# MCG-NJU/MeMOTR

Hardware: AMD Instinct MI355X
Metric: train_frames_per_sec (higher is better)
Workload: dtype f32

## Files before the change

### memotr_amd/csrc/clip_ops.hip

```cpp
#include <hip/hip_runtime.h>
#include <stdint.h>
#include <stdio.h>

#include <atomic>

#include "../../include/clip_ops_hip.h"
#include "assign_core.h"

namespace {

thread_local char g_err[256] = {0};

int fail(int code, const char *msg) {
    snprintf(g_err, sizeof(g_err), "%s", msg);
    return code;
}

int check_launch(const char *what) {
    const hipError_t e = hipGetLastError();
    if (e != hipSuccess) {
        snprintf(g_err, sizeof(g_err), "%s: %s", what, hipGetErrorString(e));
        return (int)e;
    }
    g_err[0] = 0;
// ... 330 lines not shown
        a.y += __shfl_xor(a.y, o, 64);
        a.z += __shfl_xor(a.z, o, 64);
        a.w += __shfl_xor(a.w, o, 64);
    }
    if ((threadIdx.x & 63) == 0) s_w[threadIdx.x >> 6] = a;
    __syncthreads();
    if (threadIdx.x == 0) *reinterpret_cast<f32x4_t *>(out + c) = (s_w[0] + s_w[1]) + (s_w[2] + s_w[3]);
}

__device__ __forceinline__ float colsum_ld(const float *x, long i) { return x[i]; }
__device__ __forceinline__ float colsum_ld(const uint16_t *x, long i) {
    return __uint_as_float(((unsigned)x[i]) << 16);
}

template <typename TX>
__global__ __launch_bounds__(256) void colsum_partial_kernel(const TX *__restrict__ x, long rows, int cols,
                                                            int chunk_rows, float *__restrict__ partial) {
    __shared__ float s_part[8][33];
    const int tx = threadIdx.x & 31, ty = threadIdx.x >> 5;
    const int c = blockIdx.x * 32 + tx;
    const long r0 = (long)blockIdx.y * chunk_rows;
    const long r1 = r0 + chunk_rows < rows ? r0 + chunk_rows : rows;
    float a0 = 0.f, a1 = 0.f, a2 = 0.f, a3 = 0.f;
    if (c < cols) {
        long r = r0 + ty;
        for (; r + 24 < r1; r += 32) {
            a0 += colsum_ld(x, r * cols + c);
            a1 += colsum_ld(x, (r + 8) * cols + c);
            a2 += colsum_ld(x, (r + 16) * cols + c);
            a3 += colsum_ld(x, (r + 24) * cols + c);
        }
        for (; r < r1; r += 8) a0 += colsum_ld(x, r * cols + c);
    }
    s_part[ty][tx] = (a0 + a1) + (a2 + a3);
    __syncthreads();
    if (ty == 0 && c < cols) {
        float t = s_part[0][tx];
#pragma unroll
        for (int i = 1; i < 8; ++i) t += s_part[i][tx];
        partial[(long)blockIdx.y * cols + c] = t;
    }
}

__device__ __forceinline__ void colsum_st(float *x, long i, float v) { x[i] = v; }

template <typename TX>
__global__ __launch_bounds__(256) void relu_bwd_colsum_partial_kernel(const TX *__restrict__ g, const TX *__restrict__ y,
                                                                     long rows, int cols, int chunk_rows,
                                                                     TX *__restrict__ g2, float *__restrict__ partial) {
    __shared__ float s_part[8][33];
    const int tx = threadIdx.x & 31, ty = threadIdx.x >> 5;
    const int c = blockIdx.x * 32 + tx;
    const long r0 = (long)blockIdx.y * chunk_rows;
    const long r1 = r0 + chunk_rows < rows ? r0 + chunk_rows : rows;
    float a0 = 0.f, a1 = 0.f, a2 = 0.f, a3 = 0.f;
    if (c < cols) {
        long r = r0 + ty;
        for (; r + 24 < r1; r += 32) {
            const long i0 = r * cols + c, i1 = (r + 8) * cols + c, i2 = (r + 16) * cols + c, i3 = (r + 24) * cols + c;
            const float v0 = colsum_ld(y, i0) <= 0.f ? 0.f : colsum_ld(g, i0);
            const float v1 = colsum_ld(y, i1) <= 0.f ? 0.f : colsum_ld(g, i1);
            const float v2 = colsum_ld(y, i2) <= 0.f ? 0.f : colsum_ld(g, i2);
            const float v3 = colsum_ld(y, i3) <= 0.f ? 0.f : colsum_ld(g, i3);
            colsum_st(g2, i0, v0); colsum_st(g2, i1, v1); colsum_st(g2, i2, v2); colsum_st(g2, i3, v3);
            a0 += v0; a1 += v1; a2 += v2; a3 += v3;
        }
        for (; r < r1; r += 8) {
            const long i0 = r * cols + c;
            const float v0 = colsum_ld(y, i0) <= 0.f ? 0.f : colsum_ld(g, i0);
            colsum_st(g2, i0, v0);
            a0 += v0;
        }
    }
    s_part[ty][tx] = (a0 + a1) + (a2 + a3);
    __syncthreads();
    if (ty == 0 && c < cols) {
        float t = s_part[0][tx];
#pragma unroll
        for (int i = 1; i < 8; ++i) t += s_part[i][tx];
        partial[(long)blockIdx.y * cols + c] = t;
    }
}

constexpr int kLanes = 16;
constexpr int kRows = 256 / kLanes;
constexpr int kHd = 32;
constexpr int kPitch = 36;

__device__ __forceinline__ void load_row32(const float *p, float *r) {
#pragma unroll
    for (int i = 0; i < 8; ++i) {
        const f32x4_t v = *reinterpret_cast<const f32x4_t *>(p + 4 * i);
        r[4 * i] = v.x; r[4 * i + 1] = v.y; r[4 * i + 2] = v.z; r[4 * i + 3] = v.w;
    }
}

__device__ __forceinline__ float dot32(const float *a, const float *lds_row) {
    float s0 = 0.f, s1 = 0.f;
#pragma unroll
    for (int i = 0; i < 8; ++i) {
        const f32x4_t v = *reinterpret_cast<const f32x4_t *>(lds_row + 4 * i);
        s0 = fmaf(a[4 * i], v.x, s0);
        s1 = fmaf(a[4 * i + 1], v.y, s1);
        s0 = fmaf(a[4 * i + 2], v.z, s0);
        s1 = fmaf(a[4 * i + 3], v.w, s1);
    }
    return s0 + s1;
}

__device__ __forceinline__ void axpy32(float *acc, float w, const float *lds_row) {
#pragma unroll
    for (int i = 0; i < 8; ++i) {
        const f32x4_t v = *reinterpret_cast<const f32x4_t *>(lds_row + 4 * i);
        acc[4 * i] = fmaf(w, v.x, acc[4 * i]);
        acc[4 * i + 1] = fmaf(w, v.y, acc[4 * i + 1]);
        acc[4 * i + 2] = fmaf(w, v.z, acc[4 * i + 2]);
        acc[4 * i + 3] = fmaf(w, v.w, acc[4 * i + 3]);
    }
}

__device__ __forceinline__ float sum8l(float x) {
#pragma unroll
    for (int o = 1; o < kLanes; o <<= 1) x += __shfl_xor(x, o, 64);
    return x;
}
__device__ __forceinline__ float max8l(float x) {
#pragma unroll
    for (int o = 1; o < kLanes; o <<= 1) x = fmaxf(x, __shfl_xor(x, o, 64));
    return x;
}

__device__ __forceinline__ void stage_rows(float *dst, const float *src, long rs, int L) {
    for (int i = threadIdx.x; i < L * 8; i += blockDim.x) {
        const int r = i >> 3, c = (i & 7) * 4;
        *reinterpret_cast<f32x4_t *>(dst + r * kPitch + c) = *reinterpret_cast<const f32x4_t *>(src + r * rs + c);
    }
}

__global__ __launch_bounds__(256) void mha_fwd_kernel(const float *__restrict__ q, const float *__restrict__ k,
                                                     const float *__restrict__ v, long q_bs, long q_rs, long k_bs,
                                                     long k_rs, long v_bs, long v_rs,
                                                     const uint8_t *__restrict__ key_mask, int H, int L, float scale,
                                                     float *__restrict__ out, float *__restrict__ lse) {
    extern __shared__ __attribute__((aligned(16))) float s_mem[];
    float *Ks = s_mem, *Vs = s_mem + (size_t)L * kPitch;
    const int h = blockIdx.y, b = blockIdx.z;
    stage_rows(Ks, k + b * k_bs + h * kHd, k_rs, L);
    stage_rows(Vs, v + b * v_bs + h * kHd, v_rs, L);
    __syncthreads();
    const int row = blockIdx.x * kRows + threadIdx.x / kLanes, sub = threadIdx.x % kLanes;
    const bool row_ok = row < L;
    const int rowc = row_ok ? row : L - 1;
    float qr[kHd];
    load_row32(q + b * q_bs + rowc * q_rs + h * kHd, qr);
#pragma unroll
    for (int i = 0; i < kHd; ++i) qr[i] *= scale;
    const uint8_t *mk = key_mask ? key_mask + (long)b * L : nullptr;
    float m = -INFINITY, l = 0.f, acc[kHd];
#pragma unroll
    for (int i = 0; i < kHd; ++i) acc[i] = 0.f;
    for (int j = sub; j < L; j += kLanes) {
        if (mk && mk[j]) continue;
        const float s = dot32(qr, Ks + j * kPitch);
        const float m_new = fmaxf(m, s);
        const float corr = expf(m - m_new), p = expf(s - m_new);
        l = l * corr + p;
#pragma unroll
        for (int i = 0; i < kHd; ++i) acc[i] *= corr;
        axpy32(acc, p, Vs + j * kPitch);
        m = m_new;
    }
    const float M = max8l(m);
    const float w = (m == -INFINITY) ? 0.f : expf(m - M);
    const float Lsum = sum8l(l * w);
    const float inv = 1.f / Lsum;
    float *o = out + ((long)b * L + rowc) * (H * kHd) + h * kHd;
#pragma unroll
    for (int i = 0; i < kHd; ++i) {
        const float t = sum8l(acc[i] * w) * inv;
        if (row_ok && (i >> 2) == sub) o[i] = t;
    }
    if (row_ok && sub == 0) lse[((long)b * H + h) * L + row] = M + logf(Lsum);
}

__global__ __launch_bounds__(256) void mha_bwd_q_kernel(const float *__restrict__ q, const float *__restrict__ k,
                                                       const float *__restrict__ v, long q_bs, long q_rs, long k_bs,
                                                       long k_rs, long v_bs, long v_rs,
                                                       const uint8_t *__restrict__ key_mask,
                                                       const float *__restrict__ out, const float *__restrict__ lse,
                                                       const float *__restrict__ go, int H, int L, float scale,
                                                       float *__restrict__ gq, long gq_bs, long gq_rs) {
    extern __shared__ __attribute__((aligned(16))) float s_mem[];
    float *Ks = s_mem, *Vs = s_mem + (size_t)L * kPitch;
    const int h = blockIdx.y, b = blockIdx.z;
    stage_rows(Ks, k + b * k_bs + h * kHd, k_rs, L);
    stage_rows(Vs, v + b * v_bs + h * kHd, v_rs, L);
    __syncthreads();
    const int row = blockIdx.x * kRows + threadIdx.x / kLanes, sub = threadIdx.x % kLanes;
    const bool row_ok = row < L;
    const int rowc = row_ok ? row : L - 1;
    float qr[kHd], gr[kHd], acc[kHd];
    load_row32(q + b * q_bs + rowc * q_rs + h * kHd, qr);
    const long orow = ((long)b * L + rowc) * (H * kHd) + h * kHd;
    load_row32(go + orow, gr);
    float D = 0.f;
    {
        float orr[kHd];
        load_row32(out + orow, orr);
#pragma unroll
        for (int i = 0; i < kHd; ++i) D = fmaf(gr[i], orr[i], D);
    }
#pragma unroll
    for (int i = 0; i < kHd; ++i) { qr[i] *= scale; acc[i] = 0.f; }
    const float ls = lse[((long)b * H + h) * L + rowc];
    const uint8_t *mk = key_mask ? key_mask + (long)b * L : nullptr;
    for (int j = sub; j < L; j += kLanes) {
        if (mk && mk[j]) continue;
        const float p = expf(dot32(qr, Ks + j * kPitch) - ls);
        const float ds = p * (dot32(gr, Vs + j * kPitch) - D);
        axpy32(acc, ds, Ks + j * kPitch);
    }
    float *g = gq + b * gq_bs + rowc * gq_rs + h * kHd;
#pragma unroll
    for (int i = 0; i < kHd; ++i) {
        const float t = sum8l(acc[i]) * scale;
        if (row_ok && (i >> 2) == sub) g[i] = t;
    }
}

__global__ __launch_bounds__(256) void mha_bwd_kv_kernel(const float *__restrict__ q, const float *__restrict__ k,
                                                        const float *__restrict__ v, long q_bs, long q_rs, long k_bs,
                                                        long k_rs, long v_bs, long v_rs,
                                                        const uint8_t *__restrict__ key_mask,
                                                        const float *__restrict__ out, const float *__restrict__ lse,
                                                        const float *__restrict__ go, int H, int L, float scale,
                                                        float *__restrict__ gk, long gk_bs, long gk_rs,
                                                        float *__restrict__ gv, long gv_bs, long gv_rs) {
    extern __shared__ __attribute__((aligned(16))) float s_mem[];
    float *Qs = s_mem, *Gs = s_mem + (size_t)L * kPitch;
    float *s_lse = Gs + (size_t)L * kPitch, *s_D = s_lse + L;
    const int h = blockIdx.y, b = blockIdx.z;
    stage_rows(Qs, q + b * q_bs + h * kHd, q_rs, L);
    stage_rows(Gs, go + (long)b * L * (H * kHd) + h * kHd, (long)H * kHd, L);
    for (int i = threadIdx.x; i < L; i += blockDim.x) s_lse[i] = lse[((long)b * H + h) * L + i];
    __syncthreads();
    for (int i = threadIdx.x; i < L; i += blockDim.x) {
        const float *o = out + ((long)b * L + i) * (H * kHd) + h * kHd;
        float d = 0.f;
#pragma unroll
        for (int c = 0; c < kHd; ++c) d = fmaf(Gs[i * kPitch + c], o[c], d);
        s_D[i] = d;
    }
    __syncthreads();
    const int row = blockIdx.x * kRows + threadIdx.x / kLanes, sub = threadIdx.x % kLanes;
    const bool row_ok = row < L;
    const int rowc = row_ok ? row : L - 1;
    const bool dead = key_mask && key_mask[(long)b * L + rowc];
    float kr[kHd], vr[kHd], ak[kHd], av[kHd];
    load_row32(k + b * k_bs + rowc * k_rs + h * kHd, kr);
    load_row32(v + b * v_bs + rowc * v_rs + h * kHd, vr);
#pragma unroll
    for (int i = 0; i < kHd; ++i) { kr[i] *= scale; ak[i] = 0.f; av[i] = 0.f; }
    if (!dead) {
        for (int i = sub; i < L; i += kLanes) {
            const float p = expf(dot32(kr, Qs + i * kPitch) - s_lse[i]);
            const float ds = p * (dot32(vr, Gs + i * kPitch) - s_D[i]);
            axpy32(av, p, Gs + i * kPitch);
            axpy32(ak, ds, Qs + i * kPitch);
        }
    }
    float *pk = gk + b * gk_bs + rowc * gk_rs + h * kHd, *pv = gv + b * gv_bs + rowc * gv_rs + h * kHd;
#pragma unroll
    for (int i = 0; i < kHd; ++i) {
        const float tk = sum8l(ak[i]) * scale, tv = sum8l(av[i]);
        if (row_ok && (i >> 2) == sub) {
            pk[i] = tk;
            pv[i] = tv;
        }
    }
}

int allow_lds(const void *kernel, size_t lds, std::atomic<unsigned long long> &done) {
    if (lds <= 64 * 1024) return 0;
    int dev = 0;
    (void)hipGetDevice(&dev);
    const unsigned long long bit = 1ull << (dev & 63);
    if (done.load(std::memory_order_acquire) & bit) return 0;
    const hipError_t e = hipFuncSetAttribute(kernel, hipFuncAttributeMaxDynamicSharedMemorySize, 160 * 1024 - 2048);
    if (e != hipSuccess) {
        snprintf(g_err, sizeof(g_err), "hipFuncSetAttribute: %s", hipGetErrorString(e));
        return (int)e;
    }
    done.fetch_or(bit, std::memory_order_release);
    return 0;
}

std::atomic<unsigned long long> g_lds_fwd{0}, g_lds_bq{0}, g_lds_bkv{0};

int mha_check(const void *q, const void *k, const void *v, int B, int H, int L) {
    if (B < 0 || H <= 0 || L < 0) return fail(1, "clipops_mha: bad dimension");
    if (L > CLIPOPS_MHA_MAX_L) return fail(2, "clipops_mha: L exceeds CLIPOPS_MHA_MAX_L");
    if ((long)B * L > 0 && (!q || !k || !v)) return fail(1, "clipops_mha: null pointer");
    return 0;
}

__device__ __forceinline__ float wave_sum64(float x) {
#pragma unroll
    for (int o = 32; o > 0; o >>= 1) x += __shfl_xor(x, o, 64);
    return x;
}

__global__ __launch_bounds__(256) void add_layer_norm_fwd_kernel(const float *__restrict__ x,
                                                                const float *__restrict__ res,
                                                                const float *__restrict__ gamma,
                                                                const float *__restrict__ beta, long rows, float eps,
                                                                float *__restrict__ sum, float *__restrict__ y,
                                                                float *__restrict__ stats) {
    const int lane = threadIdx.x & 63;
    const long row = (long)blockIdx.x * 4 + (threadIdx.x >> 6);
    if (row >= rows) return;
    const long off = row * CLIPOPS_LN_COLS + lane * 4;
    const f32x4_t a = *reinterpret_cast<const f32x4_t *>(x + off);
    const f32x4_t b = *reinterpret_cast<const f32x4_t *>(res + off);
    const f32x4_t s = a + b;
    *reinterpret_cast<f32x4_t *>(sum + off) = s;
    const float mean = wave_sum64((s.x + s.y) + (s.z + s.w)) * (1.f / CLIPOPS_LN_COLS);
    const f32x4_t d = s - mean;
    const float var = wave_sum64((d.x * d.x + d.y * d.y) + (d.z * d.z + d.w * d.w)) * (1.f / CLIPOPS_LN_COLS);
    const float rstd = rsqrtf(var + eps);
    const f32x4_t g = *reinterpret_cast<const f32x4_t *>(gamma + lane * 4);
    const f32x4_t be = *reinterpret_cast<const f32x4_t *>(beta + lane * 4);
    *reinterpret_cast<f32x4_t *>(y + off) = (d * rstd) * g + be;
    if (lane == 0) {
        stats[2 * row] = mean;
        stats[2 * row + 1] = rstd;
    }
}

__global__ __launch_bounds__(256) void add_layer_norm_bwd_kernel(const float *__restrict__ gy,
                                                                const float *__restrict__ sum,
                                                                const float *__restrict__ stats,
                                                                const float *__restrict__ gamma, long rows,
                                                                int chunk_rows, float *__restrict__ gsum,
                                                                float *__restrict__ partial) {
    __shared__ f32x4_t s_acc[4][2][64];
    const int lane = threadIdx.x & 63, wave = threadIdx.x >> 6;
    const f32x4_t gm = *reinterpret_cast<const f32x4_t *>(gamma + lane * 4);
    f32x4_t acc_g = {0.f, 0.f, 0.f, 0.f}, acc_b = {0.f, 0.f, 0.f, 0.f};
    const long r0 = (long)blockIdx.x * chunk_rows;
    const long r1 = r0 + chunk_rows < rows ? r0 + chunk_rows : rows;
    for (long row = r0 + wave; row < r1; row += 4) {
        const long off = row * CLIPOPS_LN_COLS + lane * 4;
        const f32x4_t g = *reinterpret_cast<const f32x4_t *>(gy + off);
        const f32x4_t s = *reinterpret_cast<const f32x4_t *>(sum + off);
        const float mean = stats[2 * row], rstd = stats[2 * row + 1];
        const f32x4_t xh = (s - mean) * rstd;
        const f32x4_t gh = g * gm;
        const float c1 = wave_sum64((gh.x + gh.y) + (gh.z + gh.w)) * (1.f / CLIPOPS_LN_COLS);
        const float c2 = wave_sum64((gh.x * xh.x + gh.y * xh.y) + (gh.z * xh.z + gh.w * xh.w)) * (1.f / CLIPOPS_LN_COLS);
        *reinterpret_cast<f32x4_t *>(gsum + off) = (gh - c1 - xh * c2) * rstd;
        acc_g += g * xh;
        acc_b += g;
    }
    s_acc[wave][0][lane] = acc_g;
    s_acc[wave][1][lane] = acc_b;
    __syncthreads();
    if (wave < 2) {
        const f32x4_t t = (s_acc[0][wave][lane] + s_acc[1][wave][lane]) + (s_acc[2][wave][lane] + s_acc[3][wave][lane]);
        *reinterpret_cast<f32x4_t *>(partial + (long)blockIdx.x * 2 * CLIPOPS_LN_COLS + wave * CLIPOPS_LN_COLS + lane * 4) = t;
    }
}

struct WaveLanes {
    int lane;
    template <typename F>
    __device__ __forceinline__ assign::ScanBest scan(int n, F &&body) const {
        assign::ScanBest mine = assign::scan_empty();
        for (int it = lane; it < n; it += 64) body(it, mine);
#pragma unroll
        for (int off = 32; off >= 1; off >>= 1) {
// ... 33 lines not shown
    return (int)(g > 4096 ? 4096 : g);
}


__device__ __forceinline__ float sr_bf16(uint16_t h) { return __uint_as_float((unsigned)h << 16); }
__device__ __forceinline__ uint16_t sr_to_bf16(float f) {
    unsigned u = __float_as_uint(f);
    if ((u & 0x7fffffffu) > 0x7f800000u) return (uint16_t)((u >> 16) | 0x40u);
    return (uint16_t)((u + 0x7fffu + ((u >> 16) & 1u)) >> 16);
}

template <bool RES>
__global__ __launch_bounds__(256) void shift_relu_f32_kernel(float *__restrict__ x, const float *__restrict__ shift,
                                                             const float *__restrict__ res, long planes, int C, long HW,
                                                             int vec) {
    for (long plane = blockIdx.y; plane < planes; plane += gridDim.y) {
        const float b = shift[plane % C];
        float *xp = x + plane * HW;
        const float *rp = RES ? res + plane * HW : nullptr;
        if (vec) {
            const long n4 = HW >> 2;
            for (long i = (long)blockIdx.x * blockDim.x + threadIdx.x; i < n4; i += (long)gridDim.x * blockDim.x) {
                float4 v = reinterpret_cast<float4 *>(xp)[i];
                if (RES) {
                    const float4 r = reinterpret_cast<const float4 *>(rp)[i];
                    v.x = (v.x + b) + r.x; v.y = (v.y + b) + r.y; v.z = (v.z + b) + r.z; v.w = (v.w + b) + r.w;
                } else {
                    v.x += b; v.y += b; v.z += b; v.w += b;
                }
                v.x = v.x < 0.f ? 0.f : v.x; v.y = v.y < 0.f ? 0.f : v.y;
                v.z = v.z < 0.f ? 0.f : v.z; v.w = v.w < 0.f ? 0.f : v.w;
                reinterpret_cast<float4 *>(xp)[i] = v;
            }
        } else {
            for (long i = (long)blockIdx.x * blockDim.x + threadIdx.x; i < HW; i += (long)gridDim.x * blockDim.x) {
                float v = xp[i] + b;
                if (RES) v += rp[i];
                xp[i] = v < 0.f ? 0.f : v;
            }
        }
    }
}

template <bool RES>
__global__ __launch_bounds__(256) void shift_relu_bf16_kernel(uint16_t *__restrict__ x, const float *__restrict__ shift,
                                                              const uint16_t *__restrict__ res, long planes, int C,
                                                              long HW, int vec) {
    for (long plane = blockIdx.y; plane < planes; plane += gridDim.y) {
        const float b = sr_bf16(sr_to_bf16(shift[plane % C]));
        uint16_t *xp = x + plane * HW;
        const uint16_t *rp = RES ? res + plane * HW : nullptr;
        if (vec) {
            const long n8 = HW >> 3;
            for (long i = (long)blockIdx.x * blockDim.x + threadIdx.x; i < n8; i += (long)gridDim.x * blockDim.x) {
                uint4 v = reinterpret_cast<uint4 *>(xp)[i];
                uint4 r = {0u, 0u, 0u, 0u};
                if (RES) r = reinterpret_cast<const uint4 *>(rp)[i];
                unsigned *vw = reinterpret_cast<unsigned *>(&v);
                const unsigned *rw = reinterpret_cast<const unsigned *>(&r);
#pragma unroll
                for (int k = 0; k < 4; ++k) {
                    float lo = sr_bf16((uint16_t)(vw[k] & 0xffffu)) + b, hi = sr_bf16((uint16_t)(vw[k] >> 16)) + b;
                    if (RES) {
                        lo = sr_bf16(sr_to_bf16(lo)) + sr_bf16((uint16_t)(rw[k] & 0xffffu));
                        hi = sr_bf16(sr_to_bf16(hi)) + sr_bf16((uint16_t)(rw[k] >> 16));
                    }
                    lo = lo < 0.f ? 0.f : lo;
                    hi = hi < 0.f ? 0.f : hi;
                    vw[k] = (unsigned)sr_to_bf16(lo) | ((unsigned)sr_to_bf16(hi) << 16);
                }
                reinterpret_cast<uint4 *>(xp)[i] = v;
            }
        } else {
            for (long i = (long)blockIdx.x * blockDim.x + threadIdx.x; i < HW; i += (long)gridDim.x * blockDim.x) {
                float v = sr_bf16(xp[i]) + b;
                if (RES) v = sr_bf16(sr_to_bf16(v)) + sr_bf16(rp[i]);
                xp[i] = sr_to_bf16(v < 0.f ? 0.f : v);
            }
        }
    }
}


typedef float lb_f32x16 __attribute__((ext_vector_type(16)));

#ifndef MSDA_LB_U
#define MSDA_LB_U 4
#endif
constexpr int LB_U = MSDA_LB_U;

template <bool GX, bool RELU>
__device__ __forceinline__ void linear_bwd_tile(const float *__restrict__ g, const float *__restrict__ y,
                                                const float *__restrict__ Bp, int M, int N, int K, int OUT, int i0, int j0,
                                                float *__restrict__ C, float *__restrict__ gb, float (*s_c)[16][64],
                                                float (*s_b)[32]) {
    const int lane = threadIdx.x & 63, wave = threadIdx.x >> 6;
    const int i = i0 + (lane & 31), j = j0 + (lane & 31), kq = (lane >> 5) * 4;
    const bool iok = i < M, jok = j < N;
    const int chunks = (K + 7) / 8, per = (chunks + 3) / 4;
    const int c_lo = wave * per, c_hi = (c_lo + per) < chunks ? (c_lo + per) : chunks;
    const bool vec = GX && (OUT % 4 == 0);
    lb_f32x16 acc = {0.f, 0.f, 0.f, 0.f, 0.f, 0.f, 0.f, 0.f, 0.f, 0.f, 0.f, 0.f, 0.f, 0.f, 0.f, 0.f};
    float bsum = 0.f;
    for (int c = c_lo; c < c_hi; c += LB_U) {
        float a[LB_U][4], b[LB_U][4], m[LB_U][4];
#pragma unroll
        for (int u = 0; u < LB_U; ++u) {
            const int k0 = (c + u) * 8 + kq;
            const bool cok = c + u < c_hi;
            if (vec) {
                float4 av = {0.f, 0.f, 0.f, 0.f}, mv = {1.f, 1.f, 1.f, 1.f};
                if (cok && iok && k0 < K) {
                    av = *reinterpret_cast<const float4 *>(g + (long)i * OUT + k0);
                    if (RELU) mv = *reinterpret_cast<const float4 *>(y + (long)i * OUT + k0);
                }
                a[u][0] = av.x; a[u][1] = av.y; a[u][2] = av.z; a[u][3] = av.w;
                m[u][0] = mv.x; m[u][1] = mv.y; m[u][2] = mv.z; m[u][3] = mv.w;
            }
#pragma unroll
            for (int q = 0; q < 4; ++q) {
                const int k = k0 + q;
                const bool kok = cok && k < K;
                if (!vec) {
                    const long idx = GX ? (long)i * OUT + k : (long)k * OUT + i;
                    a[u][q] = (iok && kok) ? g[idx] : 0.f;
                    m[u][q] = (RELU && iok && kok) ? y[idx] : 1.f;
                }
                b[u][q] = (jok && kok) ? Bp[(long)k * N + j] : 0.f;
            }
        }
#pragma unroll
        for (int u = 0; u < LB_U; ++u) {
#pragma unroll
            for (int q = 0; q < 4; ++q) {
                const float av = RELU ? (m[u][q] <= 0.f ? 0.f : a[u][q]) : a[u][q];
                acc = __builtin_amdgcn_mfma_f32_32x32x2f32(av, b[u][q], acc, 0, 0, 0);
                bsum += av;
            }
        }
    }
#pragma unroll
    for (int r = 0; r < 16; ++r) s_c[wave][r][lane] = acc[r];
    bsum += __shfl_xor(bsum, 32, 64);
    if (lane < 32) s_b[wave][lane] = bsum;
    __syncthreads();
#pragma unroll
    for (int rr = 0; rr < 4; ++rr) {
        const int r = wave * 4 + rr;
        const float v = (s_c[0][r][lane] + s_c[1][r][lane]) + (s_c[2][r][lane] + s_c[3][r][lane]);
        const int row = i0 + (r & 3) + 8 * (r >> 2) + 4 * (lane >> 5);
        if (row < M && jok) C[(long)row * N + j] = v;
    }
    if (!GX && gb != nullptr && j0 == 0 && wave == 0 && lane < 32 && i0 + lane < M)
        gb[i0 + lane] = (s_b[0][lane] + s_b[1][lane]) + (s_b[2][lane] + s_b[3][lane]);
}

template <bool RELU>
__global__ __launch_bounds__(256) void linear_bwd_kernel(const float *__restrict__ g, const float *__restrict__ y,
                                                         const float *__restrict__ x, const float *__restrict__ w,
                                                         int R, int IN, int OUT, float *__restrict__ gx,
                                                         float *__restrict__ gw, float *__restrict__ gb, int n_gx,
                                                         int gx_tj, int gw_tj) {
    __shared__ float s_c[4][16][64];
    __shared__ float s_b[4][32];
    const int tile = blockIdx.x;
    if (tile < n_gx) {
        linear_bwd_tile<true, RELU>(g, y, w, R, IN, OUT, OUT, (tile / gx_tj) * 32, (tile % gx_tj) * 32, gx, nullptr, s_c, s_b);
    } else {
// ... 223 lines not shown
    return check_launch("inverse_sigmoid_bwd_kernel");
}

int clipops_refine_boxes_fwd_f32(const float *delta, const float *ref, long n, float eps, float *out, void *stream) {
    if (n < 0) return fail(1, "clipops_refine_boxes_fwd_f32: negative count");
    if (n == 0) { g_err[0] = 0; return 0; }
    if (!delta || !ref || !out) return fail(1, "clipops_refine_boxes_fwd_f32: null pointer");
    hipLaunchKernelGGL(refine_boxes_fwd_kernel, dim3(grid_for(n)), dim3(256), 0, (hipStream_t)stream, delta, ref, n,
                       eps, out);
    return check_launch("refine_boxes_fwd_kernel");
}

int clipops_refine_boxes_bwd_f32(const float *out, const float *ref, const float *grad_out, long n, float eps,
                                 float *grad_delta, float *grad_ref, void *stream) {
    if (n < 0) return fail(1, "clipops_refine_boxes_bwd_f32: negative count");
    if (n == 0) { g_err[0] = 0; return 0; }
    if (!out || !ref || !grad_out || !grad_delta) return fail(1, "clipops_refine_boxes_bwd_f32: null pointer");
    hipLaunchKernelGGL(refine_boxes_bwd_kernel, dim3(grid_for(n)), dim3(256), 0, (hipStream_t)stream, out, ref,
                       grad_out, n, eps, grad_delta, grad_ref);
    return check_launch("refine_boxes_bwd_kernel");
}

int clipops_colsum_f32(const float *x, long rows, int cols, float *out, void *stream) {
    if (rows < 0 || cols < 0) return fail(1, "clipops_colsum_f32: bad dimension");
    if (cols == 0) { g_err[0] = 0; return 0; }
    if (!out || (rows > 0 && !x)) return fail(1, "clipops_colsum_f32: null pointer");
    if (cols % 4 == 0 && rows <= 2048 && (((uintptr_t)x | (uintptr_t)out) & 15) == 0) {
        hipLaunchKernelGGL(colsum_quad_kernel, dim3(cols / 4), dim3(256), 0, (hipStream_t)stream, x, rows, cols, out);
        return check_launch("colsum_quad_kernel");
    }
    hipLaunchKernelGGL(colsum_kernel, dim3((cols + 31) / 32), dim3(256), 0, (hipStream_t)stream, x, rows, cols, out);
    return check_launch("colsum_kernel");
}

int clipops_colsum_partial_f32(const float *x, long rows, int cols, int chunk_rows, float *partial, void *stream) {
    if (rows < 0 || cols < 0 || chunk_rows <= 0) return fail(1, "clipops_colsum_partial_f32: bad dimension");
    if (cols == 0 || rows == 0) { g_err[0] = 0; return 0; }
    if (!x || !partial) return fail(1, "clipops_colsum_partial_f32: null pointer");
    const long chunks = (rows + chunk_rows - 1) / chunk_rows;
    if (chunks > 65535) return fail(1, "clipops_colsum_partial_f32: too many chunks");
    hipLaunchKernelGGL(colsum_partial_kernel<float>, dim3((cols + 31) / 32, (unsigned)chunks), dim3(256), 0,
                       (hipStream_t)stream, x, rows, cols, chunk_rows, partial);
    return check_launch("colsum_partial_kernel");
}

int clipops_colsum_partial_bf16(const uint16_t *x, long rows, int cols, int chunk_rows, float *partial, void *stream) {
    if (rows < 0 || cols < 0 || chunk_rows <= 0) return fail(1, "clipops_colsum_partial_bf16: bad dimension");
    if (cols == 0 || rows == 0) { g_err[0] = 0; return 0; }
    if (!x || !partial) return fail(1, "clipops_colsum_partial_bf16: null pointer");
    const long chunks = (rows + chunk_rows - 1) / chunk_rows;
    if (chunks > 65535) return fail(1, "clipops_colsum_partial_bf16: too many chunks");
    hipLaunchKernelGGL(colsum_partial_kernel<uint16_t>, dim3((cols + 31) / 32, (unsigned)chunks), dim3(256), 0,
                       (hipStream_t)stream, x, rows, cols, chunk_rows, partial);
    return check_launch("colsum_partial_kernel<bf16>");
}

static int relu_bwd_colsum_check(const void *g, const void *y, const void *g2, const void *partial, long rows, int cols,
                                 int chunk_rows, long *chunks) {
    if (rows < 0 || cols < 0 || chunk_rows <= 0) return fail(1, "clipops_relu_bwd_colsum_partial: bad dimension");
    *chunks = (rows + chunk_rows - 1) / chunk_rows;
    if (cols == 0 || rows == 0) return 0;
    if (!g || !y || !g2 || !partial) return fail(1, "clipops_relu_bwd_colsum_partial: null pointer");
    if (*chunks > 65535) return fail(1, "clipops_relu_bwd_colsum_partial: too many chunks");
    return 0;
}

int clipops_relu_bwd_colsum_partial_f32(const float *g, const float *y, long rows, int cols, int chunk_rows, float *g2,
                                        float *partial, void *stream) {
    long chunks = 0;
    if (relu_bwd_colsum_check(g, y, g2, partial, rows, cols, chunk_rows, &chunks)) return 1;
    if (cols == 0 || rows == 0) { g_err[0] = 0; return 0; }
    hipLaunchKernelGGL(relu_bwd_colsum_partial_kernel<float>, dim3((cols + 31) / 32, (unsigned)chunks), dim3(256), 0,
                       (hipStream_t)stream, g, y, rows, cols, chunk_rows, g2, partial);
    return check_launch("relu_bwd_colsum_partial_kernel");
}

int clipops_mha_fwd_f32(const float *q, const float *k, const float *v, long q_bs, long q_rs, long k_bs, long k_rs,
                        long v_bs, long v_rs, const uint8_t *key_mask, int B, int H, int L, float scale, float *out,
                        float *lse, void *stream) {
    int rc = mha_check(q, k, v, B, H, L);
    if (rc) return rc;
    if ((long)B * L == 0) { g_err[0] = 0; return 0; }
    if (!out || !lse) return fail(1, "clipops_mha_fwd_f32: null pointer");
    const size_t lds = (size_t)2 * L * kPitch * sizeof(float);
    if ((rc = allow_lds(reinterpret_cast<const void *>(mha_fwd_kernel), lds, g_lds_fwd))) return rc;
    hipLaunchKernelGGL(mha_fwd_kernel, dim3((L + kRows - 1) / kRows, H, B), dim3(256), lds, (hipStream_t)stream, q, k, v, q_bs,
                       q_rs, k_bs, k_rs, v_bs, v_rs, key_mask, H, L, scale, out, lse);
    return check_launch("mha_fwd_kernel");
}

int clipops_mha_bwd_f32(const float *q, const float *k, const float *v, long q_bs, long q_rs, long k_bs, long k_rs,
                        long v_bs, long v_rs, const uint8_t *key_mask, const float *out, const float *lse,
                        const float *grad_out, int B, int H, int L, float scale, float *grad_q, long gq_bs, long gq_rs,
                        float *grad_k, long gk_bs, long gk_rs, float *grad_v, long gv_bs, long gv_rs, void *stream) {
    int rc = mha_check(q, k, v, B, H, L);
    if (rc) return rc;
    if ((long)B * L == 0) { g_err[0] = 0; return 0; }
    if (!out || !lse || !grad_out || !grad_q || !grad_k || !grad_v) return fail(1, "clipops_mha_bwd_f32: null pointer");
    const size_t lds_q = (size_t)2 * L * kPitch * sizeof(float);
    const size_t lds_kv = lds_q + (size_t)2 * L * sizeof(float);
    if ((rc = allow_lds(reinterpret_cast<const void *>(mha_bwd_q_kernel), lds_q, g_lds_bq))) return rc;
    if ((rc = allow_lds(reinterpret_cast<const void *>(mha_bwd_kv_kernel), lds_kv, g_lds_bkv))) return rc;
    const dim3 grid((L + kRows - 1) / kRows, H, B);
    hipLaunchKernelGGL(mha_bwd_q_kernel, grid, dim3(256), lds_q, (hipStream_t)stream, q, k, v, q_bs, q_rs, k_bs, k_rs,
                       v_bs, v_rs, key_mask, out, lse, grad_out, H, L, scale, grad_q, gq_bs, gq_rs);
    if ((rc = check_launch("mha_bwd_q_kernel"))) return rc;
    hipLaunchKernelGGL(mha_bwd_kv_kernel, grid, dim3(256), lds_kv, (hipStream_t)stream, q, k, v, q_bs, q_rs, k_bs, k_rs,
                       v_bs, v_rs, key_mask, out, lse, grad_out, H, L, scale, grad_k, gk_bs, gk_rs, grad_v, gv_bs, gv_rs);
    return check_launch("mha_bwd_kv_kernel");
}

int clipops_add_layer_norm_fwd_f32(const float *x, const float *res, const float *gamma, const float *beta, long rows,
                                   float eps, float *sum, float *y, float *stats, void *stream) {
    if (rows < 0) return fail(1, "clipops_add_layer_norm_fwd_f32: negative row count");
    if (rows == 0) { g_err[0] = 0; return 0; }
    if (!x || !res || !gamma || !beta || !sum || !y || !stats) return fail(1, "clipops_add_layer_norm_fwd_f32: null pointer");
    hipLaunchKernelGGL(add_layer_norm_fwd_kernel, dim3((unsigned)((rows + 3) / 4)), dim3(256), 0, (hipStream_t)stream, x,
                       res, gamma, beta, rows, eps, sum, y, stats);
    return check_launch("add_layer_norm_fwd_kernel");
}

int clipops_add_layer_norm_bwd_f32(const float *grad_y, const float *sum, const float *stats, const float *gamma,
                                   long rows, int chunk_rows, float *grad_sum, float *partial, void *stream) {
    if (rows < 0 || chunk_rows <= 0) return fail(1, "clipops_add_layer_norm_bwd_f32: bad dimension");
    if (rows == 0) { g_err[0] = 0; return 0; }
    if (!grad_y || !sum || !stats || !gamma || !grad_sum || !partial)
        return fail(1, "clipops_add_layer_norm_bwd_f32: null pointer");
    hipLaunchKernelGGL(add_layer_norm_bwd_kernel, dim3((unsigned)((rows + chunk_rows - 1) / chunk_rows)), dim3(256), 0,
                       (hipStream_t)stream, grad_y, sum, stats, gamma, rows, chunk_rows, grad_sum, partial);
    return check_launch("add_layer_norm_bwd_kernel");
}

int clipops_assign_f32(const float *cost, long stride_problem, long stride_row, long stride_col, int n_problems,
                       int n_rows, int n_cols, int32_t *row_ind, int32_t *col_ind, int32_t *status, void *stream) {
    if (n_problems < 0 || n_rows < 0 || n_cols < 0) return fail(1, "clipops_assign_f32: bad dimension");
    if (n_problems == 0 || n_rows == 0 || n_cols == 0) { g_err[0] = 0; return 0; }
    if (!cost || !row_ind || !col_ind) return fail(1, "clipops_assign_f32: null pointer");
    const int nr = n_rows < n_cols ? n_rows : n_cols, nc = n_rows < n_cols ? n_cols : n_rows;
    if (nc > CLIPOPS_ASSIGN_MAX_DIM) return fail(2, "clipops_assign_f32: problem exceeds CLIPOPS_ASSIGN_MAX_DIM");
    const size_t lds = (assign::work_bytes(nr, nc) + 15) & ~(size_t)15;
    if (lds > 64 * 1024) {
        static std::atomic<size_t> allowed{0};
        if (lds > 160 * 1024) return fail(2, "clipops_assign_f32: problem does not fit the LDS of a CU");
        if (lds > allowed.load()) {
            if (hipFuncSetAttribute(reinterpret_cast<const void *>(assign_kernel),
                                    hipFuncAttributeMaxDynamicSharedMemorySize, 160 * 1024) != hipSuccess) {
                (void)hipGetLastError();
                return fail(3, "clipops_assign_f32: hipFuncSetAttribute(MaxDynamicSharedMemorySize) failed");
            }
            allowed.store(160 * 1024);
        }
    }
    hipLaunchKernelGGL(assign_kernel, dim3(n_problems), dim3(64), lds, (hipStream_t)stream, cost, stride_problem,
                       stride_row, stride_col, n_rows, n_cols, row_ind, col_ind, status);
    return check_launch("assign_kernel");
}

static int shift_relu_check(const void *x, const void *shift, long planes, int C, long HW, const char *who) {
    if (planes < 0 || C <= 0 || HW < 0) return fail(1, who);
    if (planes && HW && (!x || !shift)) return fail(1, who);
    return 0;
}

int clipops_shift_relu_f32(float *x, const float *shift, const float *res, long planes, int C, long HW, void *stream) {
    if (shift_relu_check(x, shift, planes, C, HW, "clipops_shift_relu_f32: bad argument")) return 1;
    if (planes == 0 || HW == 0) { g_err[0] = 0; return 0; }
    const int vec = (HW % 4 == 0) && ((uintptr_t)x % 16 == 0) && (!res || (uintptr_t)res % 16 == 0);
    const long per = vec ? HW / 4 : HW;
    const dim3 grid((unsigned)((per + 1023) / 1024 > 64 ? 64 : (per + 1023) / 1024 < 1 ? 1 : (per + 1023) / 1024),
                    (unsigned)(planes > 65535 ? 65535 : planes));
    if (res) hipLaunchKernelGGL(shift_relu_f32_kernel<true>, grid, dim3(256), 0, (hipStream_t)stream, x, shift, res, planes, C, HW, vec);
    else hipLaunchKernelGGL(shift_relu_f32_kernel<false>, grid, dim3(256), 0, (hipStream_t)stream, x, shift, res, planes, C, HW, vec);
    return check_launch("shift_relu_f32_kernel");
}

int clipops_shift_relu_bf16(uint16_t *x, const float *shift, const uint16_t *res, long planes, int C, long HW, void *stream) {
    if (shift_relu_check(x, shift, planes, C, HW, "clipops_shift_relu_bf16: bad argument")) return 1;
    if (planes == 0 || HW == 0) { g_err[0] = 0; return 0; }
    const int vec = (HW % 8 == 0) && ((uintptr_t)x % 16 == 0) && (!res || (uintptr_t)res % 16 == 0);
    const long per = vec ? HW / 8 : HW;
    const dim3 grid((unsigned)((per + 1023) / 1024 > 64 ? 64 : (per + 1023) / 1024 < 1 ? 1 : (per + 1023) / 1024),
                    (unsigned)(planes > 65535 ? 65535 : planes));
    if (res) hipLaunchKernelGGL(shift_relu_bf16_kernel<true>, grid, dim3(256), 0, (hipStream_t)stream, x, shift, res, planes, C, HW, vec);
    else hipLaunchKernelGGL(shift_relu_bf16_kernel<false>, grid, dim3(256), 0, (hipStream_t)stream, x, shift, res, planes, C, HW, vec);
    return check_launch("shift_relu_bf16_kernel");
}

int clipops_linear_bwd_f32(const float *grad_y, const float *y_relu, const float *x, const float *w, int rows,
                           int in_features, int out_features, float *grad_x, float *grad_w, float *grad_b,
                           void *stream) {
// ... 34 lines not shown
```

Measured before the change: 41.27.

## Rewrite fused MHA forward and backward kernels to use MFMA 32x32 tiles

Replaces the scalar per-row attention kernels, which staged all K/V of a head in LDS and used 16-lane shuffle reductions, with MFMA f32 32x32x2 matrix-core tiles. Each wave handles a strided set of 32-key tiles with register double-buffered global loads. Partial results from the four waves are merged through a small fixed LDS buffer, so the dynamic LDS sizing and opt-in attribute are no longer needed. This targets scalar FMA throughput and the LDS capacity limit for long sequences. In exchange it adds strided column loads from global memory and a cross-wave merge step.

```diff
diff --git a/memotr_amd/csrc/clip_ops.hip b/memotr_amd/csrc/clip_ops.hip
--- a/memotr_amd/csrc/clip_ops.hip
+++ b/memotr_amd/csrc/clip_ops.hip
@@ -436,59 +436,79 @@
     }
 }
 
-constexpr int kLanes = 16;
-constexpr int kRows = 256 / kLanes;
+typedef float lb_f32x16 __attribute__((ext_vector_type(16)));
+
 constexpr int kHd = 32;
-constexpr int kPitch = 36;
-
-__device__ __forceinline__ void load_row32(const float *p, float *r) {
-#pragma unroll
-    for (int i = 0; i < 8; ++i) {
+constexpr int kMT = 32;
+
+__device__ __forceinline__ int mt_row(int r, int hf) { return (r & 3) + 8 * (r >> 2) + 4 * hf; }
+
+__device__ __forceinline__ void load_half16(const float *base, long rs, int row, int L, int hf, float *r) {
+    const bool ok = row < L;
+    const float *p = base + (long)(ok ? row : L - 1) * rs + 16 * hf;
+#pragma unroll
+    for (int i = 0; i < 4; ++i) {
         const f32x4_t v = *reinterpret_cast<const f32x4_t *>(p + 4 * i);
-        r[4 * i] = v.x; r[4 * i + 1] = v.y; r[4 * i + 2] = v.z; r[4 * i + 3] = v.w;
-    }
-}
-
-__device__ __forceinline__ float dot32(const float *a, const float *lds_row) {
-    float s0 = 0.f, s1 = 0.f;
-#pragma unroll
-    for (int i = 0; i < 8; ++i) {
-        const f32x4_t v = *reinterpret_cast<const f32x4_t *>(lds_row + 4 * i);
-        s0 = fmaf(a[4 * i], v.x, s0);
-        s1 = fmaf(a[4 * i + 1], v.y, s1);
-        s0 = fmaf(a[4 * i + 2], v.z, s0);
-        s1 = fmaf(a[4 * i + 3], v.w, s1);
-    }
-    return s0 + s1;
-}
-
-__device__ __forceinline__ void axpy32(float *acc, float w, const float *lds_row) {
-#pragma unroll
-    for (int i = 0; i < 8; ++i) {
-        const f32x4_t v = *reinterpret_cast<const f32x4_t *>(lds_row + 4 * i);
-        acc[4 * i] = fmaf(w, v.x, acc[4 * i]);
-        acc[4 * i + 1] = fmaf(w, v.y, acc[4 * i + 1]);
-        acc[4 * i + 2] = fmaf(w, v.z, acc[4 * i + 2]);
-        acc[4 * i + 3] = fmaf(w, v.w, acc[4 * i + 3]);
-    }
-}
-
-__device__ __forceinline__ float sum8l(float x) {
-#pragma unroll
-    for (int o = 1; o < kLanes; o <<= 1) x += __shfl_xor(x, o, 64);
-    return x;
-}
-__device__ __forceinline__ float max8l(float x) {
-#pragma unroll
-    for (int o = 1; o < kLanes; o <<= 1) x = fmaxf(x, __shfl_xor(x, o, 64));
-    return x;
-}
-
-__device__ __forceinline__ void stage_rows(float *dst, const float *src, long rs, int L) {
-    for (int i = threadIdx.x; i < L * 8; i += blockDim.x) {
-        const int r = i >> 3, c = (i & 7) * 4;
-        *reinterpret_cast<f32x4_t *>(dst + r * kPitch + c) = *reinterpret_cast<const f32x4_t *>(src + r * rs + c);
-    }
+        r[4 * i] = ok ? v.x : 0.f; r[4 * i + 1] = ok ? v.y : 0.f; r[4 * i + 2] = ok ? v.z : 0.f; r[4 * i + 3] = ok ? v.w : 0.f;
+    }
+}
+
+__device__ __forceinline__ void load_col16(const float *base, long rs, int row0, int L, int hf, int col, float *r) {
+#pragma unroll
+    for (int k = 0; k < 16; ++k) {
+        const int row = row0 + mt_row(k, hf);
+        const float v = base[(long)(row < L ? row : L - 1) * rs + col];
+        r[k] = row < L ? v : 0.f;
+    }
+}
+
+__device__ __forceinline__ lb_f32x16 mma16(const float *a, const float *b, lb_f32x16 acc) {
+#pragma unroll
+    for (int k = 0; k < 16; ++k) acc = __builtin_amdgcn_mfma_f32_32x32x2f32(a[k], b[k], acc, 0, 0, 0);
+    return acc;
+}
+
+__device__ __forceinline__ lb_f32x16 zero16() {
+    return lb_f32x16{0.f, 0.f, 0.f, 0.f, 0.f, 0.f, 0.f, 0.f, 0.f, 0.f, 0.f, 0.f, 0.f, 0.f, 0.f, 0.f};
+}
+
+__device__ __forceinline__ unsigned live_keys16(bool dead, int hf) {
+    const unsigned long long dm = __ballot(dead);
+    unsigned live = 0;
+#pragma unroll
+    for (int r = 0; r < 16; ++r) live |= (unsigned)(~dm >> mt_row(r, hf) & 1ull) << r;
+    return live;
+}
+
+__device__ __forceinline__ f32x4_t merge_tile(float (*s_c)[16][64]) {
+    const int row = threadIdx.x >> 3, d4 = (threadIdx.x & 7) * 4;
+    const int r0 = 4 * (d4 >> 3), ln = row + 32 * ((d4 >> 2) & 1);
+    float t[4];
+#pragma unroll
+    for (int i = 0; i < 4; ++i)
+        t[i] = (s_c[0][r0 + i][ln] + s_c[1][r0 + i][ln]) + (s_c[2][r0 + i][ln] + s_c[3][r0 + i][ln]);
+    return f32x4_t{t[0], t[1], t[2], t[3]};
+}
+
+struct MhaKvTile {
+    float ka[16];
+    float vx[16];
+    float kt[16];
+    unsigned mbyte;
+};
+
+template <bool BWD>
+__device__ __forceinline__ void load_kv_tile(MhaKvTile &t, const float *kb, long k_rs, const float *vb, long v_rs,
+                                             const uint8_t *mk, int tile, int L, int hf, int col) {
+    const int key0 = tile * kMT, key = key0 + col;
+    load_half16(kb, k_rs, key, L, hf, t.ka);
+    if (BWD) {
+        load_half16(vb, v_rs, key, L, hf, t.vx);
+        load_col16(kb, k_rs, key0, L, hf, col, t.kt);
+    } else {
+        load_col16(vb, v_rs, key0, L, hf, col, t.vx);
+    }
+    t.mbyte = mk != nullptr ? mk[key < L ? key : L - 1] : 0u;
 }
 
 __global__ __launch_bounds__(256) void mha_fwd_kernel(const float *__restrict__ q, const float *__restrict__ k,
@@ -496,45 +516,68 @@
                                                      long k_rs, long v_bs, long v_rs,
                                                      const uint8_t *__restrict__ key_mask, int H, int L, float scale,
                                                      float *__restrict__ out, float *__restrict__ lse) {
-    extern __shared__ __attribute__((aligned(16))) float s_mem[];
-    float *Ks = s_mem, *Vs = s_mem + (size_t)L * kPitch;
-    const int h = blockIdx.y, b = blockIdx.z;
-    stage_rows(Ks, k + b * k_bs + h * kHd, k_rs, L);
-    stage_rows(Vs, v + b * v_bs + h * kHd, v_rs, L);
+    __shared__ float s_c[4][16][64];
+    __shared__ float s_m[4][32], s_l[4][32];
+    const int lane = threadIdx.x & 63, wave = threadIdx.x >> 6, col = lane & 31, hf = lane >> 5;
+    const int h = blockIdx.y, b = blockIdx.z, q0 = blockIdx.x * kMT;
+    const int nt = (L + kMT - 1) / kMT;
+    float qr[16];
+    load_half16(q + b * q_bs + h * kHd, q_rs, q0 + col, L, hf, qr);
+#pragma unroll
+    for (int i = 0; i < 16; ++i) qr[i] *= scale;
+    const float *kb = k + b * k_bs + h * kHd, *vb = v + b * v_bs + h * kHd;
+    const uint8_t *mk = key_mask ? key_mask + (long)b * L : nullptr;
+    float m = -INFINITY, l = 0.f;
+    lb_f32x16 o = zero16();
+    MhaKvTile cur, nxt;
+    if (wave < nt) load_kv_tile<false>(cur, kb, k_rs, vb, v_rs, mk, wave, L, hf, col);
+    for (int t = wave; t < nt; t += 4) {
+        if (t + 4 < nt) load_kv_tile<false>(nxt, kb, k_rs, vb, v_rs, mk, t + 4, L, hf, col);
+        lb_f32x16 s = mma16(cur.ka, qr, zero16());
+        const unsigned live = live_keys16(cur.mbyte != 0u || t * kMT + col >= L, hf);
+        float mx = -INFINITY;
+#pragma unroll
+        for (int r = 0; r < 16; ++r) {
+            s[r] = (live >> r & 1u) ? s[r] : -INFINITY;
+            mx = fmaxf(mx, s[r]);
+        }
+        mx = fmaxf(mx, __shfl_xor(mx, 32, 64));
+        const float m_new = fmaxf(m, mx);
+        const float base = (m_new == -INFINITY) ? 0.f : m_new;
+        const float corr = expf(m - base);
+        float p[16], psum = 0.f;
+#pragma unroll
+        for (int r = 0; r < 16; ++r) {
+            p[r] = expf(s[r] - base);
+            psum += p[r];
+        }
+        l = l * corr + psum;
+        o *= corr;
+        o = mma16(cur.vx, p, o);
+        m = m_new;
+        cur = nxt;
+    }
+    if (hf == 0) s_m[wave][col] = m;
     __syncthreads();
-    const int row = blockIdx.x * kRows + threadIdx.x / kLanes, sub = threadIdx.x % kLanes;
-    const bool row_ok = row < L;
-    const int rowc = row_ok ? row : L - 1;
-    float qr[kHd];
-    load_row32(q + b * q_bs + rowc * q_rs + h * kHd, qr);
-#pragma unroll
-    for (int i = 0; i < kHd; ++i) qr[i] *= scale;
-    const uint8_t *mk = key_mask ? key_mask + (long)b * L : nullptr;
-    float m = -INFINITY, l = 0.f, acc[kHd];
-#pragma unroll
-    for (int i = 0; i < kHd; ++i) acc[i] = 0.f;
-    for (int j = sub; j < L; j += kLanes) {
-        if (mk && mk[j]) continue;
-        const float s = dot32(qr, Ks + j * kPitch);
-        const float m_new = fmaxf(m, s);
-        const float corr = expf(m - m_new), p = expf(s - m_new);
-        l = l * corr + p;
-#pragma unroll
-        for (int i = 0; i < kHd; ++i) acc[i] *= corr;
-        axpy32(acc, p, Vs + j * kPitch);
-        m = m_new;
-    }
-    const float M = max8l(m);
+    const float M = fmaxf(fmaxf(s_m[0][col], s_m[1][col]), fmaxf(s_m[2][col], s_m[3][col]));
     const float w = (m == -INFINITY) ? 0.f : expf(m - M);
-    const float Lsum = sum8l(l * w);
+#pragma unroll
+    for (int r = 0; r < 16; ++r) s_c[wave][r][lane] = o[r] * w;
+    float lw = l * w;
+    lw += __shfl_xor(lw, 32, 64);
+    if (hf == 0) s_l[wave][col] = lw;
+    __syncthreads();
+    const int row = threadIdx.x >> 3, d4 = (threadIdx.x & 7) * 4;
+    if (q0 + row >= L) return;
+    const float Lsum = (s_l[0][row] + s_l[1][row]) + (s_l[2][row] + s_l[3][row]);
     const float inv = 1.f / Lsum;
-    float *o = out + ((long)b * L + rowc) * (H * kHd) + h * kHd;
-#pragma unroll
-    for (int i = 0; i < kHd; ++i) {
-        const float t = sum8l(acc[i] * w) * inv;
-        if (row_ok && (i >> 2) == sub) o[i] = t;
-    }
-    if (row_ok && sub == 0) lse[((long)b * H + h) * L + row] = M + logf(Lsum);
+    f32x4_t t = merge_tile(s_c);
+    t.x *= inv; t.y *= inv; t.z *= inv; t.w *= inv;
+    *reinterpret_cast<f32x4_t *>(out + ((long)b * L + q0 + row) * (H * kHd) + h * kHd + d4) = t;
+    if (d4 == 0) {
+        const float Mr = fmaxf(fmaxf(s_m[0][row], s_m[1][row]), fmaxf(s_m[2][row], s_m[3][row]));
+        lse[((long)b * H + h) * L + q0 + row] = Mr + logf(Lsum);
+    }
 }
 
 __global__ __launch_bounds__(256) void mha_bwd_q_kernel(const float *__restrict__ q, const float *__restrict__ k,
@@ -544,42 +587,75 @@
                                                        const float *__restrict__ out, const float *__restrict__ lse,
                                                        const float *__restrict__ go, int H, int L, float scale,
                                                        float *__restrict__ gq, long gq_bs, long gq_rs) {
-    extern __shared__ __attribute__((aligned(16))) float s_mem[];
-    float *Ks = s_mem, *Vs = s_mem + (size_t)L * kPitch;
-    const int h = blockIdx.y, b = blockIdx.z;
-    stage_rows(Ks, k + b * k_bs + h * kHd, k_rs, L);
-    stage_rows(Vs, v + b * v_bs + h * kHd, v_rs, L);
-    __syncthreads();
-    const int row = blockIdx.x * kRows + threadIdx.x / kLanes, sub = threadIdx.x % kLanes;
-    const bool row_ok = row < L;
-    const int rowc = row_ok ? row : L - 1;
-    float qr[kHd], gr[kHd], acc[kHd];
-    load_row32(q + b * q_bs + rowc * q_rs + h * kHd, qr);
-    const long orow = ((long)b * L + rowc) * (H * kHd) + h * kHd;
-    load_row32(go + orow, gr);
+    __shared__ float s_c[4][16][64];
+    const int lane = threadIdx.x & 63, wave = threadIdx.x >> 6, col = lane & 31, hf = lane >> 5;
+    const int h = blockIdx.y, b = blockIdx.z, q0 = blockIdx.x * kMT;
+    const int nt = (L + kMT - 1) / kMT;
+    const bool q_ok = q0 + col < L;
+    const int qi = q_ok ? q0 + col : L - 1;
+    float qr[16], gr[16];
+    load_half16(q + b * q_bs + h * kHd, q_rs, q0 + col, L, hf, qr);
+    const long o_rs = (long)H * kHd;
+    load_half16(go + (long)b * L * o_rs + h * kHd, o_rs, q0 + col, L, hf, gr);
     float D = 0.f;
     {
-        float orr[kHd];
-        load_row32(out + orow, orr);
-#pragma unroll
-        for (int i = 0; i < kHd; ++i) D = fmaf(gr[i], orr[i], D);
-    }
-#pragma unroll
-    for (int i = 0; i < kHd; ++i) { qr[i] *= scale; acc[i] = 0.f; }
-    const float ls = lse[((long)b * H + h) * L + rowc];
+        float orr[16];
+        load_half16(out + (long)b * L * o_rs + h * kHd, o_rs, q0 + col, L, hf, orr);
+#pragma unroll
+        for (int i = 0; i < 16; ++i) D = fmaf(gr[i], orr[i], D);
+        D += __shfl_xor(D, 32, 64);
+    }
+#pragma unroll
+    for (int i = 0; i < 16; ++i) qr[i] *= scale;
+    const float ls = lse[((long)b * H + h) * L + qi];
+    const float *kb = k + b * k_bs + h * kHd, *vb = v + b * v_bs + h * kHd;
     const uint8_t *mk = key_mask ? key_mask + (long)b * L : nullptr;
-    for (int j = sub; j < L; j += kLanes) {
-        if (mk && mk[j]) continue;
-        const float p = expf(dot32(qr, Ks + j * kPitch) - ls);
-        const float ds = p * (dot32(gr, Vs + j * kPitch) - D);
-        axpy32(acc, ds, Ks + j * kPitch);
-    }
-    float *g = gq + b * gq_bs + rowc * gq_rs + h * kHd;
-#pragma unroll
-    for (int i = 0; i < kHd; ++i) {
-        const float t = sum8l(acc[i]) * scale;
-        if (row_ok && (i >> 2) == sub) g[i] = t;
-    }
+    lb_f32x16 acc = zero16();
+    MhaKvTile cur, nxt;
+    if (wave < nt) load_kv_tile<true>(cur, kb, k_rs, vb, v_rs, mk, wave, L, hf, col);
+    for (int t = wave; t < nt; t += 4) {
+        if (t + 4 < nt) load_kv_tile<true>(nxt, kb, k_rs, vb, v_rs, mk, t + 4, L, hf, col);
+        const lb_f32x16 s = mma16(cur.ka, qr, zero16());
+        const lb_f32x16 dp = mma16(cur.vx, gr, zero16());
+        const unsigned live = live_keys16(cur.mbyte != 0u || t * kMT + col >= L, hf);
+        float ds[16];
+#pragma unroll
+        for (int r = 0; r < 16; ++r) ds[r] = (live >> r & 1u) ? expf(s[r] - ls) * (dp[r] - D) : 0.f;
+        acc = mma16(cur.kt, ds, acc);
+        cur = nxt;
+    }
+#pragma unroll
+    for (int r = 0; r < 16; ++r) s_c[wave][r][lane] = acc[r];
+    __syncthreads();
+    const int row = threadIdx.x >> 3, d4 = (threadIdx.x & 7) * 4;
+    if (q0 + row >= L) return;
+    f32x4_t t = merge_tile(s_c);
+    t.x *= scale; t.y *= scale; t.z *= scale; t.w *= scale;
+    *reinterpret_cast<f32x4_t *>(gq + b * gq_bs + (long)(q0 + row) * gq_rs + h * kHd + d4) = t;
+}
+
+struct MhaQTile {
+    float qa[16], ga[16];
+    float qt[16], gt[16];
+    float lse, D;
+};
+
+__device__ __forceinline__ void load_q_tile(MhaQTile &t, const float *qb, long q_rs, const float *gb, const float *ob,
+                                            long o_rs, const float *lse, int tile, int L, int hf, int col) {
+    const int i0 = tile * kMT, i = i0 + col;
+    const bool ok = i < L;
+    load_half16(qb, q_rs, i, L, hf, t.qa);
+    load_half16(gb, o_rs, i, L, hf, t.ga);
+    float orr[16];
+    load_half16(ob, o_rs, i, L, hf, orr);
+    load_col16(qb, q_rs, i0, L, hf, col, t.qt);
+    load_col16(gb, o_rs, i0, L, hf, col, t.gt);
+    const float ls = lse[ok ? i : L - 1];
+    t.lse = ok ? ls : INFINITY;
+    float d = 0.f;
+#pragma unroll
+    for (int k = 0; k < 16; ++k) d = fmaf(t.ga[k], orr[k], d);
+    t.D = d;
 }
 
 __global__ __launch_bounds__(256) void mha_bwd_kv_kernel(const float *__restrict__ q, const float *__restrict__ k,
@@ -590,66 +666,66 @@
                                                         const float *__restrict__ go, int H, int L, float scale,
                                                         float *__restrict__ gk, long gk_bs, long gk_rs,
                                                         float *__restrict__ gv, long gv_bs, long gv_rs) {
-    extern __shared__ __attribute__((aligned(16))) float s_mem[];
-    float *Qs = s_mem, *Gs = s_mem + (size_t)L * kPitch;
-    float *s_lse = Gs + (size_t)L * kPitch, *s_D = s_lse + L;
-    const int h = blockIdx.y, b = blockIdx.z;
-    stage_rows(Qs, q + b * q_bs + h * kHd, q_rs, L);
-    stage_rows(Gs, go + (long)b * L * (H * kHd) + h * kHd, (long)H * kHd, L);
-    for (int i = threadIdx.x; i < L; i += blockDim.x) s_lse[i] = lse[((long)b * H + h) * L + i];
+    __shared__ float s_c[2][4][16][64];
+    __shared__ __attribute__((aligned(16))) float s_t[2][4][2][32];
+    const int lane = threadIdx.x & 63, wave = threadIdx.x >> 6, col = lane & 31, hf = lane >> 5;
+    const int h = blockIdx.y, b = blockIdx.z, k0 = blockIdx.x * kMT;
+    const int nt = (L + kMT - 1) / kMT, iters = (nt + 3) / 4;
+    float kr[16], vr[16];
+    load_half16(k + b * k_bs + h * kHd, k_rs, k0 + col, L, hf, kr);
+    load_half16(v + b * v_bs + h * kHd, v_rs, k0 + col, L, hf, vr);
+#pragma unroll
+    for (int i = 0; i < 16; ++i) kr[i] *= scale;
+    const float *qb = q + b * q_bs + h * kHd;
+    const long o_rs = (long)H * kHd;
+    const float *gb = go + (long)b * L * o_rs + h * kHd, *ob = out + (long)b * L * o_rs + h * kHd;
+    const float *lb = lse + ((long)b * H + h) * L;
+    lb_f32x16 ak = zero16(), av = zero16();
+    MhaQTile cur, nxt;
+    load_q_tile(cur, qb, q_rs, gb, ob, o_rs, lb, wave, L, hf, col);
+    for (int it = 0; it < iters; ++it) {
+        load_q_tile(nxt, qb, q_rs, gb, ob, o_rs, lb, (it + 1) * 4 + wave, L, hf, col);
+        const float Dq = cur.D + __shfl_xor(cur.D, 32, 64);
+        float (*st)[32] = s_t[it & 1][wave];
+        if (hf == 0) { st[0][col] = cur.lse; st[1][col] = Dq; }
+        __syncthreads();
+        float lr[16], dr[16];
+#pragma unroll
+        for (int g = 0; g < 4; ++g) {
+            const f32x4_t a = *reinterpret_cast<const f32x4_t *>(&st[0][8 * g + 4 * hf]);
+            const f32x4_t d = *reinterpret_cast<const f32x4_t *>(&st[1][8 * g + 4 * hf]);
+            lr[4 * g] = a.x; lr[4 * g + 1] = a.y; lr[4 * g + 2] = a.z; lr[4 * g + 3] = a.w;
+            dr[4 * g] = d.x; dr[4 * g + 1] = d.y; dr[4 * g + 2] = d.z; dr[4 * g + 3] = d.w;
+        }
+        const lb_f32x16 s = mma16(cur.qa, kr, zero16());
+        const lb_f32x16 dp = mma16(cur.ga, vr, zero16());
+        float p[16], ds[16];
+#pragma unroll
+        for (int r = 0; r < 16; ++r) {
+            p[r] = expf(s[r] - lr[r]);
+            ds[r] = p[r] * (dp[r] - dr[r]);
+        }
+        av = mma16(cur.gt, p, av);
+        ak = mma16(cur.qt, ds, ak);
+        cur = nxt;
+    }
+#pragma unroll
+    for (int r = 0; r < 16; ++r) {
+        s_c[0][wave][r][lane] = ak[r];
+        s_c[1][wave][r][lane] = av[r];
+    }
     __syncthreads();
-    for (int i = threadIdx.x; i < L; i += blockDim.x) {
-        const float *o = out + ((long)b * L + i) * (H * kHd) + h * kHd;
-        float d = 0.f;
-#pragma unroll
-        for (int c = 0; c < kHd; ++c) d = fmaf(Gs[i * kPitch + c], o[c], d);
-        s_D[i] = d;
-    }
-    __syncthreads();
-    const int row = blockIdx.x * kRows + threadIdx.x / kLanes, sub = threadIdx.x % kLanes;
-    const bool row_ok = row < L;
-    const int rowc = row_ok ? row : L - 1;
-    const bool dead = key_mask && key_mask[(long)b * L + rowc];
-    float kr[kHd], vr[kHd], ak[kHd], av[kHd];
-    load_row32(k + b * k_bs + rowc * k_rs + h * kHd, kr);
-    load_row32(v + b * v_bs + rowc * v_rs + h * kHd, vr);
-#pragma unroll
-    for (int i = 0; i < kHd; ++i) { kr[i] *= scale; ak[i] = 0.f; av[i] = 0.f; }
-    if (!dead) {
-        for (int i = sub; i < L; i += kLanes) {
-            const float p = expf(dot32(kr, Qs + i * kPitch) - s_lse[i]);
-            const float ds = p * (dot32(vr, Gs + i * kPitch) - s_D[i]);
-            axpy32(av, p, Gs + i * kPitch);
-            axpy32(ak, ds, Qs + i * kPitch);
-        }
-    }
-    float *pk = gk + b * gk_bs + rowc * gk_rs + h * kHd, *pv = gv + b * gv_bs + rowc * gv_rs + h * kHd;
-#pragma unroll
-    for (int i = 0; i < kHd; ++i) {
-        const float tk = sum8l(ak[i]) * scale, tv = sum8l(av[i]);
-        if (row_ok && (i >> 2) == sub) {
-            pk[i] = tk;
-            pv[i] = tv;
-        }
-    }
-}
-
-int allow_lds(const void *kernel, size_t lds, std::atomic<unsigned long long> &done) {
-    if (lds <= 64 * 1024) return 0;
-    int dev = 0;
-    (void)hipGetDevice(&dev);
-    const unsigned long long bit = 1ull << (dev & 63);
-    if (done.load(std::memory_order_acquire) & bit) return 0;
-    const hipError_t e = hipFuncSetAttribute(kernel, hipFuncAttributeMaxDynamicSharedMemorySize, 160 * 1024 - 2048);
-    if (e != hipSuccess) {
-        snprintf(g_err, sizeof(g_err), "hipFuncSetAttribute: %s", hipGetErrorString(e));
-        return (int)e;
-    }
-    done.fetch_or(bit, std::memory_order_release);
-    return 0;
-}
-
-std::atomic<unsigned long long> g_lds_fwd{0}, g_lds_bq{0}, g_lds_bkv{0};
+    const int row = threadIdx.x >> 3, d4 = (threadIdx.x & 7) * 4;
+    if (k0 + row >= L) return;
+    f32x4_t tk = merge_tile(s_c[0]), tv = merge_tile(s_c[1]);
+    tk.x *= scale; tk.y *= scale; tk.z *= scale; tk.w *= scale;
+    if (key_mask && key_mask[(long)b * L + k0 + row]) {
+        tk = f32x4_t{0.f, 0.f, 0.f, 0.f};
+        tv = tk;
+    }
+    *reinterpret_cast<f32x4_t *>(gk + b * gk_bs + (long)(k0 + row) * gk_rs + h * kHd + d4) = tk;
+    *reinterpret_cast<f32x4_t *>(gv + b * gv_bs + (long)(k0 + row) * gv_rs + h * kHd + d4) = tv;
+}
 
 int mha_check(const void *q, const void *k, const void *v, int B, int H, int L) {
     if (B < 0 || H <= 0 || L < 0) return fail(1, "clipops_mha: bad dimension");
@@ -849,8 +925,6 @@
 }
 
 
-typedef float lb_f32x16 __attribute__((ext_vector_type(16)));
-
 #ifndef MSDA_LB_U
 #define MSDA_LB_U 4
 #endif
@@ -1240,9 +1314,7 @@
     if (rc) return rc;
     if ((long)B * L == 0) { g_err[0] = 0; return 0; }
     if (!out || !lse) return fail(1, "clipops_mha_fwd_f32: null pointer");
-    const size_t lds = (size_t)2 * L * kPitch * sizeof(float);
-    if ((rc = allow_lds(reinterpret_cast<const void *>(mha_fwd_kernel), lds, g_lds_fwd))) return rc;
-    hipLaunchKernelGGL(mha_fwd_kernel, dim3((L + kRows - 1) / kRows, H, B), dim3(256), lds, (hipStream_t)stream, q, k, v, q_bs,
+    hipLaunchKernelGGL(mha_fwd_kernel, dim3((L + kMT - 1) / kMT, H, B), dim3(256), 0, (hipStream_t)stream, q, k, v, q_bs,
                        q_rs, k_bs, k_rs, v_bs, v_rs, key_mask, H, L, scale, out, lse);
     return check_launch("mha_fwd_kernel");
 }
@@ -1255,15 +1327,11 @@
     if (rc) return rc;
     if ((long)B * L == 0) { g_err[0] = 0; return 0; }
     if (!out || !lse || !grad_out || !grad_q || !grad_k || !grad_v) return fail(1, "clipops_mha_bwd_f32: null pointer");
-    const size_t lds_q = (size_t)2 * L * kPitch * sizeof(float);
-    const size_t lds_kv = lds_q + (size_t)2 * L * sizeof(float);
-    if ((rc = allow_lds(reinterpret_cast<const void *>(mha_bwd_q_kernel), lds_q, g_lds_bq))) return rc;
-    if ((rc = allow_lds(reinterpret_cast<const void *>(mha_bwd_kv_kernel), lds_kv, g_lds_bkv))) return rc;
-    const dim3 grid((L + kRows - 1) / kRows, H, B);
-    hipLaunchKernelGGL(mha_bwd_q_kernel, grid, dim3(256), lds_q, (hipStream_t)stream, q, k, v, q_bs, q_rs, k_bs, k_rs,
+    const dim3 grid((L + kMT - 1) / kMT, H, B);
+    hipLaunchKernelGGL(mha_bwd_q_kernel, grid, dim3(256), 0, (hipStream_t)stream, q, k, v, q_bs, q_rs, k_bs, k_rs,
                        v_bs, v_rs, key_mask, out, lse, grad_out, H, L, scale, grad_q, gq_bs, gq_rs);
     if ((rc = check_launch("mha_bwd_q_kernel"))) return rc;
-    hipLaunchKernelGGL(mha_bwd_kv_kernel, grid, dim3(256), lds_kv, (hipStream_t)stream, q, k, v, q_bs, q_rs, k_bs, k_rs,
+    hipLaunchKernelGGL(mha_bwd_kv_kernel, grid, dim3(256), 0, (hipStream_t)stream, q, k, v, q_bs, q_rs, k_bs, k_rs,
                        v_bs, v_rs, key_mask, out, lse, grad_out, H, L, scale, grad_k, gk_bs, gk_rs, grad_v, gv_bs, gv_rs);
     return check_launch("mha_bwd_kv_kernel");
 }
```

After: 41.96 (median of 3 runs). Within noise of the previous version (+1.7%).
